# martinruenz/co-fusion

Measured on AMD Instinct MI355X. Metric: frames/sec at 640x480 (N active models) + ICP-reduce achieved HBM GB/s vs peak, higher is better.
Workload: dtype f32

## Files before the change

### co_fusion_amd/csrc/cf_device.h

```cpp
#pragma once

#include <hip/hip_runtime.h>
#include <stdint.h>

#include "cf_kernels.h"

namespace cf {

constexpr int kFixICP = 32;
constexpr int kFixRGB = 32;

__host__ __device__ inline int rgb_fix_bits(float sigma)
{
    if (sigma == -1.0f || !(sigma >= 2.0f)) return 8;
    union { float f; unsigned u; } v; v.f = sigma;
    const int F = 8 + 2 * ((int)((v.u >> 23) & 255u) - 127);
    return F > 32 ? 32 : F;
}
constexpr int kFixSO3 = 12;
constexpr int kSE3Words = 32;
constexpr int kSO3Words = 16;

struct f3 { float x, y, z; };
struct m33 { float m[9]; };
// ... 205 lines not shown

__device__ __forceinline__ void gram_wave_store(int* wl, const gram_v16i& acc, int lane)
{
#pragma unroll
    for (int g = 0; g < 4; g++)
#pragma unroll
        for (int a = 0; a < 3; a++) wl[(3 * g + a) * 64 + lane] = acc[4 * g + a];
}
__device__ __forceinline__ void gram_block_commit(const int* lds, bool has, int lane, int wave, int nwaves,
                                                  unsigned long long* __restrict__ dst )
{
    __shared__ int s_has[16];
    if (lane == 0) s_has[wave] = has ? 1 : 0;
    __syncthreads();
    if (wave != 0) return;
    gram_v16i c;
#pragma unroll
    for (int r = 0; r < 16; r++) c[r] = 0;
    bool any = false;
    for (int w = 0; w < nwaves; w++) {
        if (!s_has[w]) continue;
        any = true;
        const int* src = lds + w * kGramWaveDwords + lane;
#pragma unroll
        for (int g = 0; g < 4; g++)
#pragma unroll
            for (int a = 0; a < 3; a++) c[4 * g + a] += src[(3 * g + a) * 64];
    }
    if (!any) return;
    const unsigned long long v = gram_wave_finish(c, lane);
    const int word = gram_word_of_lane(lane);
    if (word >= 0 && v != 0) atomicAdd(&dst[word], v);
}

__device__ __forceinline__ void det_sincos(double x, double* s, double* c)
{
    const double two_over_pi = 0.63661977236758134308;
    const double pio2_1 = 1.57079632673412561417e+00;
    const double pio2_1t = 6.07710050650619224932e-11;
    double fn = rint(x * two_over_pi);
    double r = (x - fn * pio2_1) - fn * pio2_1t;
    long long n = (long long)fn;
    double r2 = r * r;
    double sp = -1.0 / 355687428096000.0;
    sp = sp * r2 + 1.0 / 1307674368000.0;
    sp = sp * r2 - 1.0 / 6227020800.0;
    sp = sp * r2 + 1.0 / 39916800.0;
    sp = sp * r2 - 1.0 / 362880.0;
    sp = sp * r2 + 1.0 / 5040.0;
    sp = sp * r2 - 1.0 / 120.0;
    sp = sp * r2 + 1.0 / 6.0;
    double sr = r - r * r2 * sp;
    double cp = 1.0 / 20922789888000.0;
    cp = cp * r2 - 1.0 / 87178291200.0;
    cp = cp * r2 + 1.0 / 479001600.0;
    cp = cp * r2 - 1.0 / 3628800.0;
    cp = cp * r2 + 1.0 / 40320.0;
    cp = cp * r2 - 1.0 / 720.0;
    cp = cp * r2 + 1.0 / 24.0;
    cp = cp * r2 - 1.0 / 2.0;
    double cr = 1.0 + r2 * cp;
    switch ((int)(n & 3)) {
        case 0: *s = sr; *c = cr; break;
        case 1: *s = cr; *c = -sr; break;
        case 2: *s = -sr; *c = -cr; break;
        default: *s = -cr; *c = sr; break;
    }
}

__device__ inline void rodrigues(const double w[3], double R[9])
{
    double rx = w[0], ry = w[1], rz = w[2];
    double theta = sqrt(rx * rx + ry * ry + rz * rz);
    R[0] = 1; R[1] = 0; R[2] = 0; R[3] = 0; R[4] = 1; R[5] = 0; R[6] = 0; R[7] = 0; R[8] = 1;
    if (theta >= 2.2204460492503131e-16) {
        double s, c;
        det_sincos(theta, &s, &c);
        double c1 = 1.0 - c;
        double itheta = 1.0 / theta;
        rx *= itheta; ry *= itheta; rz *= itheta;
        const double rrt[9] = {rx * rx, rx * ry, rx * rz, rx * ry, ry * ry, ry * rz, rx * rz, ry * rz, rz * rz};
        const double rx_[9] = {0, -rz, ry, rz, 0, -rx, -ry, rx, 0};
        const double I[9] = {1, 0, 0, 0, 1, 0, 0, 0, 1};
        for (int k = 0; k < 9; k++) R[k] = c * I[k] + c1 * rrt[k] + s * rx_[k];
    }
}

template <typename T>
__device__ inline void inv33(const T a[9], T o[9])
{
    T c00 = a[4] * a[8] - a[5] * a[7];
    T c01 = a[5] * a[6] - a[3] * a[8];
    T c02 = a[3] * a[7] - a[4] * a[6];
    T det = a[0] * c00 + a[1] * c01 + a[2] * c02;
    T id = (T)1 / det;
    o[0] = c00 * id;
    o[1] = (a[2] * a[7] - a[1] * a[8]) * id;
    o[2] = (a[1] * a[5] - a[2] * a[4]) * id;
    o[3] = c01 * id;
    o[4] = (a[0] * a[8] - a[2] * a[6]) * id;
    o[5] = (a[2] * a[3] - a[0] * a[5]) * id;
    o[6] = c02 * id;
    o[7] = (a[1] * a[6] - a[0] * a[7]) * id;
    o[8] = (a[0] * a[4] - a[1] * a[3]) * id;
}

template <typename T>
__device__ inline void mul33(const T a[9], const T b[9], T o[9])
{
    for (int i = 0; i < 3; i++)
        for (int j = 0; j < 3; j++)
            o[i * 3 + j] = a[i * 3 + 0] * b[0 * 3 + j] + a[i * 3 + 1] * b[1 * 3 + j] + a[i * 3 + 2] * b[2 * 3 + j];
}

__device__ inline void mul44(const double a[16], const double b[16], double o[16])
{
    for (int i = 0; i < 4; i++)
        for (int j = 0; j < 4; j++) {
            double s = a[i * 4 + 0] * b[0 * 4 + j];
            s = s + a[i * 4 + 1] * b[1 * 4 + j];
            s = s + a[i * 4 + 2] * b[2 * 4 + j];
            s = s + a[i * 4 + 3] * b[3 * 4 + j];
            o[i * 4 + j] = s;
        }
}

__device__ inline void inv44_affine(const double a[16], double o[16])
{
    double L[9] = {a[0], a[1], a[2], a[4], a[5], a[6], a[8], a[9], a[10]}, Li[9];
    inv33<double>(L, Li);
    for (int i = 0; i < 3; i++) {
        o[i * 4 + 0] = Li[i * 3 + 0]; o[i * 4 + 1] = Li[i * 3 + 1]; o[i * 4 + 2] = Li[i * 3 + 2];
        o[i * 4 + 3] = -(Li[i * 3 + 0] * a[3] + Li[i * 3 + 1] * a[7] + Li[i * 3 + 2] * a[11]);
    }
    o[12] = 0; o[13] = 0; o[14] = 0; o[15] = 1;
}

template <typename T, int N>
__device__ inline void ldlt_solve(const T* Ain, const T* b, T* x, T tiny, T* ws, int* iws)
{
    T* A = ws; T* y = ws + N * N; T* d = ws + N * N + N;
    int* perm = iws;
    for (int i = 0; i < N * N; i++) A[i] = Ain[i];
    for (int i = 0; i < N; i++) perm[i] = i;
    for (int k = 0; k < N; k++) {
        int p = k;
        T best = A[k * N + k] < 0 ? -A[k * N + k] : A[k * N + k];
        for (int i = k + 1; i < N; i++) {
            T v = A[i * N + i] < 0 ? -A[i * N + i] : A[i * N + i];
            if (v > best) { best = v; p = i; }
        }
        if (p != k) {
            for (int j = 0; j < N; j++) { T t = A[k * N + j]; A[k * N + j] = A[p * N + j]; A[p * N + j] = t; }
            for (int i = 0; i < N; i++) { T t = A[i * N + k]; A[i * N + k] = A[i * N + p]; A[i * N + p] = t; }
            int t = perm[k]; perm[k] = perm[p]; perm[p] = t;
        }
        T akk = A[k * N + k];
        d[k] = akk;
        T aabs = akk < 0 ? -akk : akk;
        if (aabs > tiny) {
            for (int i = k + 1; i < N; i++) A[i * N + k] = A[i * N + k] / akk;
            for (int i = k + 1; i < N; i++)
                for (int j = k + 1; j <= i; j++) {
                    A[i * N + j] = A[i * N + j] - A[i * N + k] * akk * A[j * N + k];
                    A[j * N + i] = A[i * N + j];
                }
        } else {
            for (int i = k + 1; i < N; i++) A[i * N + k] = 0;
        }
    }
    for (int i = 0; i < N; i++) {
        T s = b[perm[i]];
        for (int j = 0; j < i; j++) s = s - A[i * N + j] * y[j];
        y[i] = s;
    }
    for (int i = 0; i < N; i++) {
        T aabs = d[i] < 0 ? -d[i] : d[i];
        y[i] = (aabs > tiny) ? y[i] / d[i] : (T)0;
    }
    for (int i = N - 1; i >= 0; i--) {
        T s = y[i];
        for (int j = i + 1; j < N; j++) s = s - A[j * N + i] * y[j];
        y[i] = s;
    }
    for (int i = 0; i < N; i++) x[perm[i]] = y[i];
}

__device__ __forceinline__ double readlane_f64(double v, int lane)
{
    const int lo = __builtin_amdgcn_readlane(__double2loint(v), lane);
    const int hi = __builtin_amdgcn_readlane(__double2hiint(v), lane);
    return __hiloint2double(hi, lo);
}

__device__ __forceinline__ double bpermute_f64(double v, int byte_addr)
{
    const int lo = __builtin_amdgcn_ds_bpermute(byte_addr, __double2loint(v));
    const int hi = __builtin_amdgcn_ds_bpermute(byte_addr, __double2hiint(v));
    return __hiloint2double(hi, lo);
}
__device__ __forceinline__ void ldlt_solve6_wave(double a, double* x, double tiny, int lane)
{
    const bool isB = lane >= 36 && lane < 42;
    const int i = (lane < 36) ? lane / 6 : (isB ? lane - 36 : 0), j = (lane < 36) ? lane % 6 : (isB ? 6 : 0);
    int perm[6] = {0, 1, 2, 3, 4, 5};
    double d[6];
#pragma unroll
    for (int k = 0; k < 6; k++) {
        int p = 5;
        {
            double dq[6];
#pragma unroll
            for (int q = k; q < 6; q++) dq[q] = __builtin_fabs(readlane_f64(a, q * 7));
            double M = dq[k];
#pragma unroll
            for (int q = k + 1; q < 6; q++) M = __builtin_fmax(M, dq[q]);
#pragma unroll
            for (int q = 5; q >= k; q--) p = (dq[q] == M) ? q : p;
        }
        p = __builtin_amdgcn_readfirstlane(p);
        if (p != k) {
            const int si = (i == k) ? p : ((i == p) ? k : i), sj = (j == k) ? p : ((j == p) ? k : j);
            a = bpermute_f64(a, (isB ? 36 + si : (si > sj ? si : sj) * 6 + (si > sj ? sj : si)) * 4);
            const int pk = perm[k];
            int pp = pk;
#pragma unroll
            for (int q = k + 1; q < 6; q++)
                if (q == p) { pp = perm[q]; perm[q] = pk; }
            perm[k] = pp;
        }
        const double akk = readlane_f64(a, k * 7);
        d[k] = akk;
        const double aabs = akk < 0 ? -akk : akk;
        const bool pivot_ok = aabs > tiny;
        if (j == k && i > k) a = pivot_ok ? a / akk : 0.0;
        const double lik = bpermute_f64(a, (i * 6 + k) * 4);
        const double ljk = bpermute_f64(a, (j * 6 + k) * 4);
        const double yk = readlane_f64(a, 36 + k);
        if (isB) { if (i > k) a = a - lik * yk; }
        else if (pivot_ok && i > k && j > k && j <= i) a = a - lik * akk * ljk;
    }
    double y[6];
#pragma unroll
    for (int r = 0; r < 6; r++) y[r] = readlane_f64(a, 36 + r);
    {
        double yn = y[0], dn = d[0];
#pragma unroll
        for (int r = 1; r < 6; r++) if (lane == r) { yn = y[r]; dn = d[r]; }
        const double aabs = dn < 0 ? -dn : dn;
        const double q = (aabs > tiny) ? yn / dn : 0.0;
#pragma unroll
        for (int r = 0; r < 6; r++) y[r] = readlane_f64(q, r);
    }
#pragma unroll
    for (int r = 5; r >= 0; r--) {
        double s = y[r];
#pragma unroll
        for (int c = r + 1; c < 6; c++) s = s - readlane_f64(a, c * 6 + r) * y[c];
        y[r] = s;
    }
    if (lane == 0) {
#pragma unroll
        for (int r = 0; r < 6; r++) x[perm[r]] = y[r];
    }
}


__device__ __forceinline__ float fix_to_f32(long long q, int F) { return (float)ldexp((double)q, -F); }

}
// ... 1 lines not shown
```

### co_fusion_amd/csrc/track_reduce.hip

```cpp
#include "cf_device.h"
#include "cf_kernels.h"
#include "track_prep_dev.h"
#include "track_sums_dev.h"

namespace cf {

__device__ __forceinline__ int idiv(int n, IDiv d) { return (int)(__umulhi((unsigned)n, d.M) >> d.s); }

struct IcpProj { f3 vcurr_g; int g; int inb; int ux, uy; };

__device__ __forceinline__ IcpProj icp_project(const m33& Rcurr, const f3& tcurr, const m33& Rprev_inv, const f3& tprev, const cf_cam& intr,
                                               int cols, int rows, f3 vcurr)
{
    IcpProj o;
    o.vcurr_g = mul(Rcurr, vcurr) + tcurr;
    const f3 vcurr_cp = mul(Rprev_inv, o.vcurr_g - tprev);
    const int ux = f2i_rn(vcurr_cp.x * intr.fx / vcurr_cp.z + intr.cx);
    const int uy = f2i_rn(vcurr_cp.y * intr.fy / vcurr_cp.z + intr.cy);
    o.inb = !(ux < 0 || uy < 0 || ux >= cols || uy >= rows || vcurr_cp.z < 0);
    o.g = o.inb ? uy * cols + ux : 0;
    o.ux = o.inb ? ux : 0; o.uy = o.inb ? uy : 0;
    return o;
}

// ... 695 lines not shown
        gn.rgb_acc[m] = rgb_args[0].m[m].rgb_acc;
        gn.od_host[m] = h_states ? h_states[m] : nullptr;
    }
    const bool slots = mode != 0;
    bool any_culled = false;
    for (int m = 0; m < n; m++) any_culled = any_culled || (icp_args[0].m[m].cull && icp_args[0].m[m].err);
    const bool err_aside = icp && any_culled;
    bool hook_failed = false;
    for (int i = 2; i >= 0; i--) {
        const int N = (width >> i) * (height >> i);
        for (int j = 0; j < iterations[i]; j++) {
            const bool last_of_level = (j == iterations[i] - 1);
            int next_level = i;
            if (last_of_level) {
                next_level = i - 1;
                while (next_level >= 0 && iterations[next_level] == 0) next_level--;
            }
            RgbArgs ra = rgb_args[i];
            ra.compact = slots ? 1 : 0;
            ra.slot_px = cfg.threads * 4;
            {
                const bool timed = prof && prof->enabled && i == 0 && prof->used + 4 <= prof->capacity;
                IcpArgs a = icp_args[i];
                a.flags = (i == 0 && last_of_level) ? (err_aside ? 3 : 1) : 0;
                launch_icp_rgbres(s, cfg, a, ra, icp, rgb, n, i, timed ? prof->events[prof->used] : nullptr,
                                  timed ? prof->events[prof->used + 1] : nullptr);
                if (timed) {
                    prof->used += 2;
                    prof->bytes += (uint64_t)N * ((icp ? 24 + 24 * (uint64_t)n : 0) + (rgb ? (slots ? kRgbResidualBytesCompact : kRgbResidualBytes) * (uint64_t)n : 0));
                    prof->launches += 1;
                }
            }
            const bool err_here = err_aside && i == 0 && last_of_level;
            const bool err_with_step = err_here && rgb && slots && mode != 2;
            if (err_here && !err_with_step) {
                icp_error_surface_kernel<<<dim3((N + 255) / 256, n), 256, 0, s>>>(with_cdiv(icp_args[i]));
            }
            if (hook && hook->fn) {
                FoldArgs fa{}; int nf = 0;
                for (int m = 0; m < n; m++) if (hook->split[m]) fa.acc[nf++] = gn.icp_acc[m];
                if (nf) acc_fold_kernel<<<nf, 64, 0, s>>>(fa);
                for (int m = 0; m < n; m++)
                    if (hook->split[m] && hook->fn(hook->user, 0, gn.icp_acc[m], 32, (void*)s) != 0) hook_failed = true;
            }
            if (rgb && mode == 2) {
                const int n_slots = (N + ra.slot_px - 1) / ra.slot_px, n_quads = (n_slots + 1) / 2;
                rgb_step_solve_kernel<<<8 * n_quads * ((n + 7) / 8), 256, 0, s>>>(ra, so3_syncs, n_slots, n_quads, make_idiv(n_quads > 1 ? n_quads : 2), n,
                                                                                 cfg.gram ? -1 : kFixICP, next_level, last_of_level ? 1 : 0);
                continue;
            }
            if (rgb) {
                if (slots) {
                    const int n_slots = (N + ra.slot_px - 1) / ra.slot_px;
                    if (err_with_step) rgb_slot_step_err_kernel<<<dim3(n_slots + (N + 255) / 256, n), 256, 0, s>>>(ra, n_slots, with_cdiv(icp_args[i]));
                    else rgb_slot_step_kernel<<<dim3(n_slots, n), 256, 0, s>>>(ra, n_slots);
                }
                else rgb_step_kernel<<<dim3((N + 255) / 256, n), 256, 0, s>>>(ra);
            }
            gn_solve_kernel<<<n, 256, 0, s>>>(gn, next_level, last_of_level ? 1 : 0);
        }
    }
    return !hook_failed;
}

float replay_icp_level0(hipStream_t s, IcpLaunch cfg, const IcpArgs& a0, const RgbArgs& r0, int n, int slots, int ablate, int reps, hipEvent_t e0, hipEvent_t e1)
{
    IcpArgs a = a0; a.flags = ablate << 8;
    RgbArgs ra = r0; ra.compact = slots ? 1 : 0; ra.slot_px = cfg.threads * 4;
    for (int i = 0; i < 3; i++) launch_icp_rgbres(s, cfg, a, ra, true, true, n, 0, nullptr, nullptr);
    (void)hipEventRecord(e0, s);
    for (int i = 0; i < reps; i++) launch_icp_rgbres(s, cfg, a, ra, true, true, n, 0, nullptr, nullptr);
    (void)hipEventRecord(e1, s);
    (void)hipStreamSynchronize(s);
    float ms = 0; (void)hipEventElapsedTime(&ms, e0, e1);
    return ms * 1000.f / reps;
}

#ifdef CF_ABLATE
void trace_so3_dump(hipStream_t s)
{
    (void)hipStreamSynchronize(s);
    unsigned long long h[12][8];
    if (hipMemcpyFromSymbol(h, HIP_SYMBOL(g_so3_trace), sizeof(h)) != hipSuccess) return;
    fprintf(stderr, "[so3 trace] loop %lld ns\n", (long long)(h[11][1] - h[11][0]) * 10);
    for (int it = 0; it < 10; it++) {
        if (!h[it][0] || h[it][4] < h[it][0]) continue;
        fprintf(stderr, "[so3 trace] it %d: basis %5lld  pass %5lld  meeting %5lld  solve %5lld ns\n", it, (long long)(h[it][1] - h[it][0]) * 10,
                (long long)(h[it][2] - h[it][1]) * 10, (long long)(h[it][3] - h[it][2]) * 10, (long long)(h[it][4] - h[it][3]) * 10);
    }
    unsigned long long z[12][8] = {};
    (void)hipMemcpyToSymbol(HIP_SYMBOL(g_so3_trace), z, sizeof(z));
}
static unsigned long long* g_solve_trace_dev = nullptr;
void trace_solve_begin()
{
    if (!g_solve_trace_dev && hipMalloc(reinterpret_cast<void**>(&g_solve_trace_dev), 64 * 16 * 8) != hipSuccess) return;
    (void)hipMemset(g_solve_trace_dev, 0, 64 * 16 * 8);
    const unsigned zero = 0;
    (void)hipMemcpyToSymbol(HIP_SYMBOL(g_solve_iter), &zero, sizeof(zero));
    (void)hipMemcpyToSymbol(HIP_SYMBOL(g_solve_trace), &g_solve_trace_dev, sizeof(g_solve_trace_dev));
}
void trace_solve_end(hipStream_t s, const char* path)
{
    (void)hipStreamSynchronize(s);
    unsigned long long* none = nullptr;
    (void)hipMemcpyToSymbol(HIP_SYMBOL(g_solve_trace), &none, sizeof(none));
    if (!g_solve_trace_dev) return;
    std::vector<unsigned long long> h(64 * 16);
    (void)hipMemcpy(h.data(), g_solve_trace_dev, h.size() * 8, hipMemcpyDeviceToHost);
    FILE* f = fopen(path, "a");
    if (!f) return;
    fprintf(f, "# solve: ns from the kernel's first stamp -- loaded | totals | unpacked | LDLT | rodrigues | pose | next-iteration | write-back\n");
    for (int it = 0; it < 64; it++) {
        const unsigned long long* o = &h[(size_t)it * 16];
        if (!o[0]) continue;
        fprintf(f, "%2d", it);
        for (int k = 1; k <= 8; k++) fprintf(f, " %6lld", o[k] ? (long long)(o[k] - o[0]) * 10 : -1ll);
        fprintf(f, "\n");
    }
    fclose(f);
}
void trace_step_solve(hipStream_t s, IcpLaunch cfg, const IcpArgs& a0, const RgbArgs& r0, So3Sync* syncs, int n, const char* path)
{
    IcpArgs a = a0; a.flags = 0;
    RgbArgs ra = r0; ra.compact = 1; ra.slot_px = cfg.threads * 4;
    const int N = ra.cols * ra.rows, n_slots = (N + ra.slot_px - 1) / ra.slot_px, n_quads = (n_slots + 1) / 2, grid = 8 * n_quads * ((n + 7) / 8);
    unsigned long long* d = nullptr; unsigned long long* none = nullptr;
    if (hipMalloc(reinterpret_cast<void**>(&d), (size_t)grid * 64) != hipSuccess) return;
    FILE* f = fopen(path, "w");
    for (int rep = 0; rep < 3 && f; rep++) {
        (void)hipMemset(d, 0, (size_t)grid * 64);
        launch_icp_rgbres(s, cfg, a, ra, true, true, n, 0, nullptr, nullptr);
        (void)hipStreamSynchronize(s);
        (void)hipMemcpyToSymbol(HIP_SYMBOL(g_icp_trace), &d, sizeof(d));
        rgb_step_solve_kernel<<<grid, 256, 0, s>>>(ra, syncs, n_slots, n_quads, make_idiv(n_quads > 1 ? n_quads : 2), n, cfg.gram ? -1 : kFixICP, 0, 0);
        (void)hipStreamSynchronize(s);
        (void)hipMemcpyToSymbol(HIP_SYMBOL(g_icp_trace), &none, sizeof(none));
        std::vector<unsigned long long> h((size_t)grid * 8);
        (void)hipMemcpy(h.data(), d, h.size() * 8, hipMemcpyDeviceToHost);
        unsigned long long tmin = ~0ull;
        for (int b = 0; b < grid; b++) if (h[(size_t)b * 8] && h[(size_t)b * 8] < tmin) tmin = h[(size_t)b * 8];
        fprintf(f, "# rep %d grid %d trackers %d\n", rep, grid, n);
        for (int b = 0; b < grid; b++) {
            const unsigned long long* o = &h[(size_t)b * 8];
            if (!o[0] || o[5] == 0xffff) continue;
            auto rel = [&](unsigned long long t) { return t ? (long long)(t - tmin) * 10 : -1ll; };
            fprintf(f, "%d %d %lld %lld %lld %lld %lld\n", b, (int)o[5], rel(o[0]), rel(o[1]), rel(o[2]), rel(o[3]), rel(o[4]));
        }
    }
    if (f) fclose(f);
    (void)hipFree(d);
}
void trace_icp_level0(hipStream_t s, IcpLaunch cfg, const IcpArgs& a0, const RgbArgs& r0, int n, int slots, const char* path)
{
    IcpArgs a = a0; a.flags = 0;
    RgbArgs ra = r0; ra.compact = slots ? 1 : 0; ra.slot_px = cfg.threads * 4;
    unsigned long long* d = nullptr; unsigned long long* none = nullptr;
    const size_t cap = 1u << 16;
    if (hipMalloc(reinterpret_cast<void**>(&d), cap * 32) != hipSuccess) return;
    (void)hipMemset(d, 0, cap * 32);
    for (int i = 0; i < 2; i++) launch_icp_rgbres(s, cfg, a, ra, true, true, n, 0, nullptr, nullptr);
    (void)hipStreamSynchronize(s);
    (void)hipMemcpyToSymbol(HIP_SYMBOL(g_icp_trace), &d, sizeof(d));
    launch_icp_rgbres(s, cfg, a, ra, true, true, n, 0, nullptr, nullptr);
    (void)hipStreamSynchronize(s);
    (void)hipMemcpyToSymbol(HIP_SYMBOL(g_icp_trace), &none, sizeof(none));
    std::vector<unsigned long long> h((size_t)g_last_grid * 4);
    (void)hipMemcpy(h.data(), d, h.size() * 8, hipMemcpyDeviceToHost);
    (void)hipFree(d);
    FILE* f = fopen(path, "w");
    if (!f) return;
    unsigned long long tmin = ~0ull;
// ... 47 lines not shown
```

### co_fusion_amd/csrc/track_so3_dev.h

```cpp
#pragma once
#include "track_prep_dev.h"
#include "track_sums_dev.h"

namespace cf {

__device__ __forceinline__ void screen_box(const float* lo, const float* hi, const float* Rb, const float* tb, const float* Rcurr, const float* tcurr,
                                           cf_cam intr, float distThres, int W, int H, int lane, int (&out)[4], float (&zout)[2])
{
    const float finf = __int_as_float(0x7f800000);
    zout[0] = -finf; zout[1] = finf;
    if (!(lo[0] <= hi[0])) { out[0] = 1; out[1] = 1; out[2] = 0; out[3] = 0; return; }
    const float m = distThres * 1.01f + 1e-3f;
    const float px = (lane & 1) ? hi[0] + 3.f : lo[0] - 3.f, py = (lane & 2) ? hi[1] + 3.f : lo[1] - 3.f;
    const float znear = lo[2] - m, pz = (lane & 4) ? hi[2] + m : znear;
    const float cx_ = (px - intr.cx) / intr.fx * pz, cy_ = (py - intr.cy) / intr.fy * pz;
    const float dx = (Rb[0] * cx_ + Rb[1] * cy_ + Rb[2] * pz + tb[0]) - tcurr[0];
    const float dy = (Rb[3] * cx_ + Rb[4] * cy_ + Rb[5] * pz + tb[1]) - tcurr[1];
    const float dz = (Rb[6] * cx_ + Rb[7] * cy_ + Rb[8] * pz + tb[2]) - tcurr[2];
    const float xc = Rcurr[0] * dx + Rcurr[3] * dy + Rcurr[6] * dz;
    const float yc = Rcurr[1] * dx + Rcurr[4] * dy + Rcurr[7] * dz;
    const float zc = Rcurr[2] * dx + Rcurr[5] * dy + Rcurr[8] * dz;
    const float u = intr.fx * xc / zc + intr.cx, v = intr.fy * yc / zc + intr.cy;
    const bool bad = !(znear > 0.05f) || !(zc > 0.05f) || !is_finite(u) || !is_finite(v);
    float u0 = u, u1 = u, v0 = v, v1 = v, z0 = zc, z1 = zc;
#pragma unroll
    for (int o = 1; o < 8; o <<= 1) {
        u0 = fminf(u0, __shfl_xor(u0, o, 64)); u1 = fmaxf(u1, __shfl_xor(u1, o, 64));
        v0 = fminf(v0, __shfl_xor(v0, o, 64)); v1 = fmaxf(v1, __shfl_xor(v1, o, 64));
        z0 = fminf(z0, __shfl_xor(z0, o, 64)); z1 = fmaxf(z1, __shfl_xor(z1, o, 64));
    }
    if (__any(bad)) { out[0] = 0; out[1] = 0; out[2] = W - 1; out[3] = H - 1; return; }
    zout[0] = z0 - (1e-3f + 1e-3f * fabsf(z0)); zout[1] = z1 + (1e-3f + 1e-3f * fabsf(z1));
    const float fw = (float)(W + 16), fh = (float)(H + 16);
    out[0] = (int)floorf(fminf(fmaxf(u0, -16.f), fw)) - 3; out[1] = (int)floorf(fminf(fmaxf(v0, -16.f), fh)) - 3;
    out[2] = (int)ceilf(fminf(fmaxf(u1, -16.f), fw)) + 3; out[3] = (int)ceilf(fminf(fmaxf(v1, -16.f), fh)) + 3;
}

__device__ __forceinline__ void so3_gradient(const uint8_t* __restrict__ img, int cols, int x, int y, float& gx, float& gy)
{
    const float actu = (float)img[y * cols + x];
    float back = (float)img[y * cols + x - 1], fore = (float)img[y * cols + x + 1];
    gx = ((back + actu) / 2.0f) - ((fore + actu) / 2.0f);
    back = (float)img[(y - 1) * cols + x]; fore = (float)img[(y + 1) * cols + x];
    gy = ((back + actu) / 2.0f) - ((fore + actu) / 2.0f);
}

__device__ __forceinline__ void so3_pass(const uint8_t* __restrict__ lastImage, const uint8_t* __restrict__ nextImage,
                                         const m33& B, const m33& Ki, const float* __restrict__ krlr, int cols, int rows,
                                         unsigned long long (*lds)[16], unsigned long long* totals, int block, int blocks)
{
    constexpr float lim = (float)(1 << ((50 - kFixSO3) / 2));
    constexpr float scale = (float)(1 << kFixSO3);
    const int N = cols * rows, T = blockDim.x;
    unsigned long long acc[16];
#pragma unroll
    for (int k = 0; k < 16; k++) acc[k] = 0;
    const float a = krlr[0], b = krlr[1], c = krlr[2], d = krlr[3], e = krlr[4], f = krlr[5], g = krlr[6], h = krlr[7],
                ii = krlr[8];
    for (int k = block * T + threadIdx.x; k < N; k += blocks * T) {
        const int y = k / cols, x = k - y * cols;
        const f3 unwarped = {(float)x, (float)y, 1.0f};
        const f3 warped = mul(B, unwarped);
        const int wx = f2i_rn(warped.x / warped.z), wy = f2i_rn(warped.y / warped.z);
        if (!(wx >= 1 && wx < cols - 1 && wy >= 1 && wy < rows - 1 && x >= 1 && x < cols - 1 && y >= 1 && y < rows - 1))
            continue;
        float gnx, gny, glx, gly;
        so3_gradient(nextImage, cols, wx, wy, gnx, gny);
        so3_gradient(lastImage, cols, x, y, glx, gly);
        const float gx = (gnx + glx) / 2.0f, gy = (gny + gly) / 2.0f;
        const f3 point = mul(Ki, unwarped);
        const float z2 = point.z * point.z;
        const f3 left = {((point.z * (d * gy + a * gx)) - (gy * g * y) - (gx * g * x)) / z2,
                         ((point.z * (e * gy + b * gx)) - (gy * h * y) - (gx * h * x)) / z2,
                         ((point.z * (f * gy + c * gx)) - (gy * ii * y) - (gx * ii * x)) / z2};
        const f3 jac = cross(left, point);
        const float row[4] = {jac.x, jac.y, jac.z, -((float)nextImage[wy * cols + wx] - (float)lastImage[y * cols + x])};
        double r[4], rs[4];
#pragma unroll
        for (int q = 0; q < 4; q++) { r[q] = (double)clamp_row(row[q], lim); rs[q] = (double)(clamp_row(row[q], lim) * scale); }
#pragma unroll
        for (int p = 0; p < 3; p++)
#pragma unroll
            for (int q = 0; q < 4; q++)
                if (q >= p)
                    acc[4 * p - (p * (p - 1)) / 2 + (q - p)] += (unsigned long long)__double_as_longlong(fma(rs[p], r[q], kMagic)) - kMagicBits;
        acc[9] += (unsigned long long)__double_as_longlong(fma(rs[3], r[3], kMagic)) - kMagicBits;
        acc[10] += 1;
    }
    const int lane = threadIdx.x & 63, wave = threadIdx.x >> 6;
    const unsigned long long v = wave_reduce16_u64(acc, lane);
    if ((lane & 3) == 0) lds[wave][lane >> 2] = v;
    __syncthreads();
    if (threadIdx.x < 16) {
        unsigned long long t = 0;
        for (int w = 0; w < (T >> 6); w++) t += lds[w][threadIdx.x];
        totals[threadIdx.x] = t;
    }
    __syncthreads();
}

__device__ inline void so3_unpack(const unsigned long long* t, float A[9], float b[3], float residual[2])
{
    int shift = 0;
    for (int i = 0; i < 3; ++i)
        for (int j = i; j < 4; ++j) {
            const float value = fix_to_f32((long long)t[shift++], kFixSO3);
            if (j == 3) b[i] = value;
            else A[j * 3 + i] = A[i * 3 + j] = value;
        }
    residual[0] = fix_to_f32((long long)t[9], kFixSO3);
    residual[1] = (float)(long long)t[10];
}

__device__ inline void k_matrix(cf_cam c, double K[9])
{
    for (int i = 0; i < 9; i++) K[i] = 0;
    K[0] = c.fx; K[4] = c.fy; K[2] = c.cx; K[5] = c.cy; K[8] = 1;
}

__device__ inline void prepare_iteration(OdomDev* od, int level)
{
    double K[9], Kinv[9], Rt[16];
    k_matrix(cam_level(od->intr, level), K);
    inv33<double>(K, Kinv);
    inv44_affine(od->resultRt, Rt);
    const double R[9] = {Rt[0], Rt[1], Rt[2], Rt[4], Rt[5], Rt[6], Rt[8], Rt[9], Rt[10]};
    double tmp[9], KRK[9];
    mul33<double>(K, R, tmp);
    mul33<double>(tmp, Kinv, KRK);
    for (int k = 0; k < 9; k++) od->krkInv[k] = (float)KRK[k];
    const double tv[3] = {Rt[3], Rt[7], Rt[11]};
    for (int r = 0; r < 3; r++) od->kt[r] = (float)(K[r * 3 + 0] * tv[0] + K[r * 3 + 1] * tv[1] + K[r * 3 + 2] * tv[2]);
}

__global__ void __launch_bounds__(1024) so3_step_kernel(const uint8_t* __restrict__ lastImage,
                                                        const uint8_t* __restrict__ nextImage, m33 B, m33 Ki, m33 krlr,
                                                        int cols, int rows, unsigned long long* __restrict__ out16)
{
    __shared__ unsigned long long lds[16][16];
    __shared__ unsigned long long totals[16];
    so3_pass(lastImage, nextImage, B, Ki, krlr.m, cols, rows, lds, totals, blockIdx.x, gridDim.x);
    if (threadIdx.x < 16) out16[threadIdx.x] = totals[threadIdx.x];
}

#ifdef CF_ABLATE
__device__ unsigned long long g_so3_trace[12][8];
#define OSTAMP(it, k) do { if (lead && by == 0 && threadIdx.x == 0) g_so3_trace[it][k] = wall_clock64(); } while (0)
#else
#define OSTAMP(it, k) do {} while (0)
#endif
__global__ void __launch_bounds__(256) so3_prealign_kernel(const TrackerStates ts, So3Sync* __restrict__ syncs, int do_so3,
                                                           int first_level, int gx, int so3_blocks, const RgbPrepBatch prep, int prep_bx)
{
    if ((int)blockIdx.x >= so3_blocks) {
        const int r = (int)blockIdx.x - so3_blocks, m = r / prep_bx;
        rgb_prep_body(prep.m[m], r - m * prep_bx);
        return;
    }
    const int by = (int)blockIdx.x / gx, bxx = (int)blockIdx.x - by * gx;
    OdomDev* const god = ts.dev[by];
    So3Sync* sync = syncs + by;
    __shared__ OdomDev s_od;
    __shared__ unsigned long long lds[16][16];
    __shared__ unsigned long long totals[16];
    __shared__ float s_basis[9], s_kinv[9], s_krlr[9];
    __shared__ int s_done;
    __shared__ double s_resultR[9];
    __shared__ double s_K[9], s_Kinv[9];
    __shared__ float s_Rlr[9];
    __shared__ float s_lastError, s_lastCount;
    __shared__ double s_lastResultR[9];
    __shared__ float s_jtj[9], s_jtr[3], s_delta[3], s_fws[15];
    __shared__ int s_iws[3];
    const bool one_xcd = do_so3 && gx > 1;
    if (one_xcd && (bxx & 7) != (by & 7)) return;
    const int bx = one_xcd ? (bxx >> 3) : bxx;
    const bool lead = bx == 0;
    const unsigned G = one_xcd ? (unsigned)gx >> 3 : (unsigned)gx;
    {
        static_assert(sizeof(OdomDev) % 4 == 0, "OdomDev is staged as 32-bit words");
        constexpr int kWords = (int)(sizeof(OdomDev) / 4);
        const unsigned* __restrict__ src = reinterpret_cast<const unsigned*>(ts.host[by]);
        constexpr int kPer = (kWords + 255) / 256;
        unsigned w[kPer];
#pragma unroll
        for (int q = 0; q < kPer; q++) w[q] = ((int)threadIdx.x + 256 * q < kWords) ? src[threadIdx.x + 256 * q] : 0u;
#pragma unroll
        for (int q = 0; q < kPer; q++) if ((int)threadIdx.x + 256 * q < kWords) reinterpret_cast<unsigned*>(&s_od)[threadIdx.x + 256 * q] = w[q];
        __syncthreads();
        if (lead) for (int k = threadIdx.x; k < kWords; k += 256) reinterpret_cast<unsigned*>(god)[k] = reinterpret_cast<const unsigned*>(&s_od)[k];
        __syncthreads();
    }
    const OdomDev* const od = &s_od;
    const int L = 2, cols = od->width >> L, rows = od->height >> L;
    if (threadIdx.x == 0) {
        for (int k = 0; k < 9; k++) { s_resultR[k] = (k % 4 == 0) ? 1.0 : 0.0; s_lastResultR[k] = s_resultR[k]; s_Rlr[k] = (k % 4 == 0) ? 1.f : 0.f; }
        k_matrix(cam_level(od->intr, L), s_K);
        inv33<double>(s_K, s_Kinv);
        s_lastError = 3.402823466e+38F / 2; s_lastCount = 3.402823466e+38F / 2;
        s_done = 0;
        if (lead) { god->stats.so3_iterations = 0; god->stats.last_so3_error = 0; god->stats.last_so3_count = 0; }
    }
    __syncthreads();
    if (do_so3) {
        const uint8_t* __restrict__ lastNext = od->lastNextImage[L];
        const uint8_t* __restrict__ next = od->nextImage[L];
        OSTAMP(11, 0);
        for (int it = 0; it < 10; it++) {
            OSTAMP(it, 0);
            if (threadIdx.x == 0) {
                double tmp[9], H[9];
                mul33<double>(s_K, s_resultR, tmp);
                mul33<double>(tmp, s_Kinv, H);
                for (int k = 0; k < 9; k++) { s_basis[k] = (float)H[k]; s_kinv[k] = (float)s_Kinv[k]; s_krlr[k] = (float)tmp[k]; }
            }
            __syncthreads();
            m33 B, Ki;
            for (int k = 0; k < 9; k++) { B.m[k] = s_basis[k]; Ki.m[k] = s_kinv[k]; }
            OSTAMP(it, 1);
            so3_pass(lastNext, next, B, Ki, s_krlr, cols, rows, lds, totals, bx, (int)G);
            OSTAMP(it, 2);
            if (G > 1) {
                if (threadIdx.x < 64) {
                    unsigned long long* slot = sync->acc[it];
                    if (threadIdx.x < 11 && totals[threadIdx.x] != 0)
                        __hip_atomic_fetch_add(&slot[threadIdx.x], totals[threadIdx.x], __ATOMIC_RELAXED, __HIP_MEMORY_SCOPE_WORKGROUP);
                    asm volatile("s_waitcnt vmcnt(0)" ::: "memory");
                    if (threadIdx.x == 0) {
                        __hip_atomic_fetch_add(&sync->arrive, 1u, __ATOMIC_RELAXED, __HIP_MEMORY_SCOPE_WORKGROUP);
                        const unsigned target = (unsigned)(it + 1) * G;
                        unsigned spins = 0;
                        while (l2_read_u32(&sync->arrive) < target) {
                            if (++spins > (1u << 22)) { god->stats.fault = 1; break; }
                            __builtin_amdgcn_s_sleep(1);
                        }
                    }
                    __builtin_amdgcn_wave_barrier();
                    if (threadIdx.x < 16) totals[threadIdx.x] = l2_read_u64(&slot[threadIdx.x]);
                }
                __syncthreads();
            }
            OSTAMP(it, 3);
            if (threadIdx.x == 0) {
                float jtj[9], jtr[3], residual[2];
                so3_unpack(totals, jtj, jtr, residual);
                if (lead) god->stats.so3_iterations = it + 1;
                float err = sqrtf(residual[0]) / residual[1];
                float cnt = residual[1];
                if (err < s_lastError && (double)fabsf(s_lastError - cnt) < 0.001) {
                    s_done = 1;
                } else if ((double)err > (double)s_lastError + 0.001) {
                    err = s_lastError; cnt = s_lastCount;
                    for (int k = 0; k < 9; k++) s_resultR[k] = s_lastResultR[k];
                    s_done = 1;
                } else {
                    s_lastError = err; s_lastCount = cnt;
                    for (int k = 0; k < 9; k++) s_lastResultR[k] = s_resultR[k];
                    for (int k = 0; k < 9; k++) s_jtj[k] = jtj[k];
                    for (int k = 0; k < 3; k++) s_jtr[k] = jtr[k];
                    ldlt_solve<float, 3>(s_jtj, s_jtr, s_delta, 1.17549435e-38f, s_fws, s_iws);
                    const float delta[3] = {s_delta[0], s_delta[1], s_delta[2]};
                    const double dd[3] = {delta[0], delta[1], delta[2]};
                    double rotUpdate[9];
                    rodrigues(dd, rotUpdate);
                    float ru[9], nr[9];
                    for (int k = 0; k < 9; k++) ru[k] = (float)rotUpdate[k];
                    mul33<float>(ru, s_Rlr, nr);
                    for (int k = 0; k < 9; k++) { s_Rlr[k] = nr[k]; s_resultR[k] = nr[k]; }
                }
                if (lead) { god->stats.last_so3_error = err; god->stats.last_so3_count = cnt; }
            }
            __syncthreads();
            OSTAMP(it, 4);
            if (s_done) break;
        }
        OSTAMP(11, 1);
        if (G > 1 && threadIdx.x == 0) {
            if (__hip_atomic_fetch_add(&sync->depart, 1u, __ATOMIC_RELAXED, __HIP_MEMORY_SCOPE_WORKGROUP) == G - 1) {
                for (int it = 0; it < 10; it++)
                    for (int w = 0; w < 16; w++) sync->acc[it][w] = 0;
                sync->arrive = 0; sync->depart = 0;
            }
        }
    }
    if (lead && threadIdx.x < 64) {
        const int lane = threadIdx.x;
        unsigned key = 0;
        if (od->cull && lane < 6) { key = od->aabb_acc[lane]; od->aabb_acc[lane] = 0; }
        const float val = lane < 3 ? fkey_inv(~key) : fkey_inv(key);
        float lo[3], hi[3];
#pragma unroll
        for (int k = 0; k < 3; k++) { lo[k] = __shfl(val, k, 64); hi[k] = __shfl(val, 3 + k, 64); }
        if (__shfl((int)key, 3, 64) == 0) { lo[0] = 1.f; hi[0] = 0.f; }
        int ib[4] = {0, 0, od->width - 1, od->height - 1};
        float zb[2] = {-__int_as_float(0x7f800000), __int_as_float(0x7f800000)};
        if (od->cull) screen_box(lo, hi, od->box_R, od->box_t, od->Rcurr, od->tcurr, od->intr, od->distThres, od->width, od->height, lane, ib, zb);
        if (lane == 0) {
            for (int k = 0; k < 3; k++) { god->box_lo[k] = lo[k]; god->box_hi[k] = hi[k]; }
            for (int k = 0; k < 4; k++) god->stats.cull_box[k] = ib[k];
            god->cull_z[0] = zb[0]; god->cull_z[1] = zb[1];
        }
    }
    if (lead && threadIdx.x == 0) {
        for (int k = 0; k < 16; k++) god->resultRt[k] = (k % 5 == 0) ? 1.0 : 0.0;
        if (do_so3)
            for (int x = 0; x < 3; x++)
                for (int y = 0; y < 3; y++) god->resultRt[x * 4 + y] = s_resultR[x * 3 + y];
        god->lastRGBError = 3.402823466e+38F;
        god->level_done = 0;
        god->residual[0] = 0; god->residual[1] = 0;
        prepare_iteration(god, first_level);
        refresh_hot(god);
    }
}

}
```

Before: 916.3.

## Keep SO3 prealign state in registers and drop per-iteration serial basis step

The SO3 prealignment loop now keeps the rotation, last error and K matrices in per-thread registers of the first wave instead of shared memory. The basis update is folded into the solve step, which removes one __syncthreads and a serial thread-0 phase per iteration. A branch-free 3x3 LDLT replaces the generic shared-memory solver. The epilogue builds the hot state directly instead of re-reading global memory. It also adds trace instrumentation for prologue/epilogue timing and per-tracker iteration counts under CF_ABLATE. The risk is subtle numerical or ordering differences, for example with the sync reset that moved to the end of the kernel.

New measurement: 898.9. -1.9%, worse.

```diff
diff --git a/co_fusion_amd/csrc/cf_device.h b/co_fusion_amd/csrc/cf_device.h
--- a/co_fusion_amd/csrc/cf_device.h
+++ b/co_fusion_amd/csrc/cf_device.h
@@ -311,6 +311,7 @@
         const double rrt[9] = {rx * rx, rx * ry, rx * rz, rx * ry, ry * ry, ry * rz, rx * rz, ry * rz, rz * rz};
         const double rx_[9] = {0, -rz, ry, rz, 0, -rx, -ry, rx, 0};
         const double I[9] = {1, 0, 0, 0, 1, 0, 0, 0, 1};
+#pragma unroll
         for (int k = 0; k < 9; k++) R[k] = c * I[k] + c1 * rrt[k] + s * rx_[k];
     }
 }
@@ -337,7 +338,9 @@
 template <typename T>
 __device__ inline void mul33(const T a[9], const T b[9], T o[9])
 {
+#pragma unroll
     for (int i = 0; i < 3; i++)
+#pragma unroll
         for (int j = 0; j < 3; j++)
             o[i * 3 + j] = a[i * 3 + 0] * b[0 * 3 + j] + a[i * 3 + 1] * b[1 * 3 + j] + a[i * 3 + 2] * b[2 * 3 + j];
 }
@@ -358,6 +361,7 @@
 {
     double L[9] = {a[0], a[1], a[2], a[4], a[5], a[6], a[8], a[9], a[10]}, Li[9];
     inv33<double>(L, Li);
+#pragma unroll
     for (int i = 0; i < 3; i++) {
         o[i * 4 + 0] = Li[i * 3 + 0]; o[i * 4 + 1] = Li[i * 3 + 1]; o[i * 4 + 2] = Li[i * 3 + 2];
         o[i * 4 + 3] = -(Li[i * 3 + 0] * a[3] + Li[i * 3 + 1] * a[7] + Li[i * 3 + 2] * a[11]);
@@ -415,6 +419,62 @@
     for (int i = 0; i < N; i++) x[perm[i]] = y[i];
 }
 
+__device__ __forceinline__ void ldlt_solve3(const float (&A)[9], const float (&b)[3], float (&x)[3], float tiny)
+{
+    auto mag = [](float v) { return v < 0 ? -v : v; };
+    const float a00 = A[0], a01 = A[1], a02 = A[2], a10 = A[3], a11 = A[4], a12 = A[5], a20 = A[6], a21 = A[7], a22 = A[8];
+    const float b0 = b[0], b1 = b[1], b2 = b[2];
+    int p = 0;
+    float best = mag(a00);
+    if (mag(a11) > best) { best = mag(a11); p = 1; }
+    if (mag(a22) > best) p = 2;
+    float d0 = p == 0 ? a00 : (p == 1 ? a11 : a22);
+    float d1 = p == 1 ? a00 : a11;
+    float d2 = p == 2 ? a00 : a22;
+    float l10 = p == 0 ? a10 : (p == 1 ? a01 : a12);
+    float l20 = p == 0 ? a20 : (p == 1 ? a21 : a02);
+    float l21 = p == 0 ? a21 : (p == 1 ? a20 : a01);
+    int perm0 = p, perm1 = p == 1 ? 0 : 1, perm2 = p == 2 ? 0 : 2;
+    const float D0 = d0;
+    const bool ok0 = mag(D0) > tiny;
+    {
+        const float q10 = l10 / D0, q20 = l20 / D0;
+        const float n11 = d1 - q10 * D0 * q10, n21 = l21 - q20 * D0 * q10, n22 = d2 - q20 * D0 * q20;
+        l10 = ok0 ? q10 : 0.f; l20 = ok0 ? q20 : 0.f;
+        d1 = ok0 ? n11 : d1; l21 = ok0 ? n21 : l21; d2 = ok0 ? n22 : d2;
+    }
+    if (mag(d2) > mag(d1)) {
+        float t = d1; d1 = d2; d2 = t;
+        t = l10; l10 = l20; l20 = t;
+        const int ti = perm1; perm1 = perm2; perm2 = ti;
+    }
+    const float D1 = d1;
+    const bool ok1 = mag(D1) > tiny;
+    {
+        const float q21 = l21 / D1;
+        const float n22 = d2 - q21 * D1 * q21;
+        l21 = ok1 ? q21 : 0.f;
+        d2 = ok1 ? n22 : d2;
+    }
+    const float D2 = d2;
+    const bool ok2 = mag(D2) > tiny;
+    float y0 = perm0 == 0 ? b0 : (perm0 == 1 ? b1 : b2);
+    float y1 = perm1 == 0 ? b0 : (perm1 == 1 ? b1 : b2);
+    float y2 = perm2 == 0 ? b0 : (perm2 == 1 ? b1 : b2);
+    y1 = y1 - l10 * y0;
+    y2 = y2 - l20 * y0;
+    y2 = y2 - l21 * y1;
+    y0 = ok0 ? y0 / D0 : 0.f;
+    y1 = ok1 ? y1 / D1 : 0.f;
+    y2 = ok2 ? y2 / D2 : 0.f;
+    y1 = y1 - l21 * y2;
+    y0 = y0 - l10 * y1;
+    y0 = y0 - l20 * y2;
+    x[0] = perm0 == 0 ? y0 : (perm1 == 0 ? y1 : y2);
+    x[1] = perm0 == 1 ? y0 : (perm1 == 1 ? y1 : y2);
+    x[2] = perm0 == 2 ? y0 : (perm1 == 2 ? y1 : y2);
+}
+
 __device__ __forceinline__ double readlane_f64(double v, int lane)
 {
     const int lo = __builtin_amdgcn_readlane(__double2loint(v), lane);
diff --git a/co_fusion_amd/csrc/track_reduce.hip b/co_fusion_amd/csrc/track_reduce.hip
--- a/co_fusion_amd/csrc/track_reduce.hip
+++ b/co_fusion_amd/csrc/track_reduce.hip
@@ -801,12 +801,21 @@
     (void)hipStreamSynchronize(s);
     unsigned long long h[12][8];
     if (hipMemcpyFromSymbol(h, HIP_SYMBOL(g_so3_trace), sizeof(h)) != hipSuccess) return;
-    fprintf(stderr, "[so3 trace] loop %lld ns\n", (long long)(h[11][1] - h[11][0]) * 10);
+    fprintf(stderr, "[so3 trace] prologue %lld  loop %lld  epilogue %lld ns\n", (long long)(h[11][0] - h[11][2]) * 10, (long long)(h[11][1] - h[11][0]) * 10,
+            (long long)(h[11][3] - h[11][1]) * 10);
     for (int it = 0; it < 10; it++) {
         if (!h[it][0] || h[it][4] < h[it][0]) continue;
         fprintf(stderr, "[so3 trace] it %d: basis %5lld  pass %5lld  meeting %5lld  solve %5lld ns\n", it, (long long)(h[it][1] - h[it][0]) * 10,
                 (long long)(h[it][2] - h[it][1]) * 10, (long long)(h[it][3] - h[it][2]) * 10, (long long)(h[it][4] - h[it][3]) * 10);
     }
+    int iters[kMaxBatch];
+    if (hipMemcpyFromSymbol(iters, HIP_SYMBOL(g_so3_iters), sizeof(iters)) == hipSuccess) {
+        fprintf(stderr, "[so3 trace] iterations per tracker:");
+        for (int m = 0; m < kMaxBatch; m++) fprintf(stderr, " %d", iters[m]);
+        fprintf(stderr, "\n");
+    }
+    int zi[kMaxBatch] = {};
+    (void)hipMemcpyToSymbol(HIP_SYMBOL(g_so3_iters), zi, sizeof(zi));
     unsigned long long z[12][8] = {};
     (void)hipMemcpyToSymbol(HIP_SYMBOL(g_so3_trace), z, sizeof(z));
 }
diff --git a/co_fusion_amd/csrc/track_so3_dev.h b/co_fusion_amd/csrc/track_so3_dev.h
--- a/co_fusion_amd/csrc/track_so3_dev.h
+++ b/co_fusion_amd/csrc/track_so3_dev.h
@@ -99,10 +99,12 @@
     __syncthreads();
 }
 
-__device__ inline void so3_unpack(const unsigned long long* t, float A[9], float b[3], float residual[2])
+__device__ __forceinline__ void so3_unpack(const unsigned long long* t, float A[9], float b[3], float residual[2])
 {
     int shift = 0;
+#pragma unroll
     for (int i = 0; i < 3; ++i)
+#pragma unroll
         for (int j = i; j < 4; ++j) {
             const float value = fix_to_f32((long long)t[shift++], kFixSO3);
             if (j == 3) b[i] = value;
@@ -114,23 +116,9 @@
 
 __device__ inline void k_matrix(cf_cam c, double K[9])
 {
+#pragma unroll
     for (int i = 0; i < 9; i++) K[i] = 0;
     K[0] = c.fx; K[4] = c.fy; K[2] = c.cx; K[5] = c.cy; K[8] = 1;
-}
-
-__device__ inline void prepare_iteration(OdomDev* od, int level)
-{
-    double K[9], Kinv[9], Rt[16];
-    k_matrix(cam_level(od->intr, level), K);
-    inv33<double>(K, Kinv);
-    inv44_affine(od->resultRt, Rt);
-    const double R[9] = {Rt[0], Rt[1], Rt[2], Rt[4], Rt[5], Rt[6], Rt[8], Rt[9], Rt[10]};
-    double tmp[9], KRK[9];
-    mul33<double>(K, R, tmp);
-    mul33<double>(tmp, Kinv, KRK);
-    for (int k = 0; k < 9; k++) od->krkInv[k] = (float)KRK[k];
-    const double tv[3] = {Rt[3], Rt[7], Rt[11]};
-    for (int r = 0; r < 3; r++) od->kt[r] = (float)(K[r * 3 + 0] * tv[0] + K[r * 3 + 1] * tv[1] + K[r * 3 + 2] * tv[2]);
 }
 
 __global__ void __launch_bounds__(1024) so3_step_kernel(const uint8_t* __restrict__ lastImage,
@@ -145,9 +133,12 @@
 
 #ifdef CF_ABLATE
 __device__ unsigned long long g_so3_trace[12][8];
+__device__ int g_so3_iters[kMaxBatch];
+#define OITERS(n) do { g_so3_iters[by] = (n); } while (0)
 #define OSTAMP(it, k) do { if (lead && by == 0 && threadIdx.x == 0) g_so3_trace[it][k] = wall_clock64(); } while (0)
 #else
 #define OSTAMP(it, k) do {} while (0)
+#define OITERS(n) do {} while (0)
 #endif
 __global__ void __launch_bounds__(256) so3_prealign_kernel(const TrackerStates ts, So3Sync* __restrict__ syncs, int do_so3,
                                                            int first_level, int gx, int so3_blocks, const RgbPrepBatch prep, int prep_bx)
@@ -165,18 +156,28 @@
     __shared__ unsigned long long totals[16];
     __shared__ float s_basis[9], s_kinv[9], s_krlr[9];
     __shared__ int s_done;
-    __shared__ double s_resultR[9];
-    __shared__ double s_K[9], s_Kinv[9];
-    __shared__ float s_Rlr[9];
-    __shared__ float s_lastError, s_lastCount;
-    __shared__ double s_lastResultR[9];
-    __shared__ float s_jtj[9], s_jtr[3], s_delta[3], s_fws[15];
-    __shared__ int s_iws[3];
     const bool one_xcd = do_so3 && gx > 1;
     if (one_xcd && (bxx & 7) != (by & 7)) return;
     const int bx = one_xcd ? (bxx >> 3) : bxx;
     const bool lead = bx == 0;
     const unsigned G = one_xcd ? (unsigned)gx >> 3 : (unsigned)gx;
+    OSTAMP(11, 2);
+    float R[9] = {1.f, 0.f, 0.f, 0.f, 1.f, 0.f, 0.f, 0.f, 1.f}, lastR[9] = {1.f, 0.f, 0.f, 0.f, 1.f, 0.f, 0.f, 0.f, 1.f};
+    float lastError = 3.402823466e+38F / 2, lastCount = 3.402823466e+38F / 2;
+    double K[9], Kinv[9];
+    int so3_iterations = 0;
+    float so3_error = 0, so3_count = 0;
+    auto publish = [&](const float (&Rf)[9]) {
+        double Rd[9], tmp[9], H[9];
+#pragma unroll
+        for (int k = 0; k < 9; k++) Rd[k] = (double)Rf[k];
+        mul33<double>(K, Rd, tmp);
+        mul33<double>(tmp, Kinv, H);
+        if (threadIdx.x == 0) {
+#pragma unroll
+            for (int k = 0; k < 9; k++) { s_basis[k] = (float)H[k]; s_krlr[k] = (float)tmp[k]; }
+        }
+    };
     {
         static_assert(sizeof(OdomDev) % 4 == 0, "OdomDev is staged as 32-bit words");
         constexpr int kWords = (int)(sizeof(OdomDev) / 4);
@@ -189,18 +190,21 @@
         for (int q = 0; q < kPer; q++) if ((int)threadIdx.x + 256 * q < kWords) reinterpret_cast<unsigned*>(&s_od)[threadIdx.x + 256 * q] = w[q];
         __syncthreads();
         if (lead) for (int k = threadIdx.x; k < kWords; k += 256) reinterpret_cast<unsigned*>(god)[k] = reinterpret_cast<const unsigned*>(&s_od)[k];
-        __syncthreads();
     }
     const OdomDev* const od = &s_od;
     const int L = 2, cols = od->width >> L, rows = od->height >> L;
-    if (threadIdx.x == 0) {
-        for (int k = 0; k < 9; k++) { s_resultR[k] = (k % 4 == 0) ? 1.0 : 0.0; s_lastResultR[k] = s_resultR[k]; s_Rlr[k] = (k % 4 == 0) ? 1.f : 0.f; }
-        k_matrix(cam_level(od->intr, L), s_K);
-        inv33<double>(s_K, s_Kinv);
-        s_lastError = 3.402823466e+38F / 2; s_lastCount = 3.402823466e+38F / 2;
-        s_done = 0;
-        if (lead) { god->stats.so3_iterations = 0; god->stats.last_so3_error = 0; god->stats.last_so3_count = 0; }
-    }
+    if (do_so3 && threadIdx.x < 64) {
+        k_matrix(cam_level(od->intr, L), K);
+        inv33<double>(K, Kinv);
+        publish(R);
+        if (threadIdx.x == 0) {
+#pragma unroll
+            for (int k = 0; k < 9; k++) s_kinv[k] = (float)Kinv[k];
+            s_done = 0;
+        }
+    }
+    unsigned key = 0;
+    if (lead && od->cull && threadIdx.x < 6) key = od->aabb_acc[threadIdx.x];
     __syncthreads();
     if (do_so3) {
         const uint8_t* __restrict__ lastNext = od->lastNextImage[L];
@@ -208,13 +212,6 @@
         OSTAMP(11, 0);
         for (int it = 0; it < 10; it++) {
             OSTAMP(it, 0);
-            if (threadIdx.x == 0) {
-                double tmp[9], H[9];
-                mul33<double>(s_K, s_resultR, tmp);
-                mul33<double>(tmp, s_Kinv, H);
-                for (int k = 0; k < 9; k++) { s_basis[k] = (float)H[k]; s_kinv[k] = (float)s_Kinv[k]; s_krlr[k] = (float)tmp[k]; }
-            }
-            __syncthreads();
             m33 B, Ki;
             for (int k = 0; k < 9; k++) { B.m[k] = s_basis[k]; Ki.m[k] = s_kinv[k]; }
             OSTAMP(it, 1);
@@ -241,52 +238,49 @@
                 __syncthreads();
             }
             OSTAMP(it, 3);
-            if (threadIdx.x == 0) {
+            if (threadIdx.x < 64) {
                 float jtj[9], jtr[3], residual[2];
                 so3_unpack(totals, jtj, jtr, residual);
-                if (lead) god->stats.so3_iterations = it + 1;
+                so3_iterations = it + 1;
                 float err = sqrtf(residual[0]) / residual[1];
                 float cnt = residual[1];
-                if (err < s_lastError && (double)fabsf(s_lastError - cnt) < 0.001) {
-                    s_done = 1;
-                } else if ((double)err > (double)s_lastError + 0.001) {
-                    err = s_lastError; cnt = s_lastCount;
-                    for (int k = 0; k < 9; k++) s_resultR[k] = s_lastResultR[k];
-                    s_done = 1;
+                int done = 0;
+                if (err < lastError && (double)fabsf(lastError - cnt) < 0.001) {
+                    done = 1;
+                } else if ((double)err > (double)lastError + 0.001) {
+                    err = lastError; cnt = lastCount;
+#pragma unroll
+                    for (int k = 0; k < 9; k++) R[k] = lastR[k];
+                    done = 1;
                 } else {
-                    s_lastError = err; s_lastCount = cnt;
-                    for (int k = 0; k < 9; k++) s_lastResultR[k] = s_resultR[k];
-                    for (int k = 0; k < 9; k++) s_jtj[k] = jtj[k];
-                    for (int k = 0; k < 3; k++) s_jtr[k] = jtr[k];
-                    ldlt_solve<float, 3>(s_jtj, s_jtr, s_delta, 1.17549435e-38f, s_fws, s_iws);
-                    const float delta[3] = {s_delta[0], s_delta[1], s_delta[2]};
+                    lastError = err; lastCount = cnt;
+#pragma unroll
+                    for (int k = 0; k < 9; k++) lastR[k] = R[k];
+                    float delta[3];
+                    ldlt_solve3(jtj, jtr, delta, 1.17549435e-38f);
                     const double dd[3] = {delta[0], delta[1], delta[2]};
                     double rotUpdate[9];
                     rodrigues(dd, rotUpdate);
                     float ru[9], nr[9];
+#pragma unroll
                     for (int k = 0; k < 9; k++) ru[k] = (float)rotUpdate[k];
-                    mul33<float>(ru, s_Rlr, nr);
-                    for (int k = 0; k < 9; k++) { s_Rlr[k] = nr[k]; s_resultR[k] = nr[k]; }
+                    mul33<float>(ru, R, nr);
+#pragma unroll
+                    for (int k = 0; k < 9; k++) R[k] = nr[k];
+                    if (it < 9) publish(R);
                 }
-                if (lead) { god->stats.last_so3_error = err; god->stats.last_so3_count = cnt; }
+                so3_error = err; so3_count = cnt;
+                if (threadIdx.x == 0) s_done = done;
             }
             __syncthreads();
             OSTAMP(it, 4);
             if (s_done) break;
         }
         OSTAMP(11, 1);
-        if (G > 1 && threadIdx.x == 0) {
-            if (__hip_atomic_fetch_add(&sync->depart, 1u, __ATOMIC_RELAXED, __HIP_MEMORY_SCOPE_WORKGROUP) == G - 1) {
-                for (int it = 0; it < 10; it++)
-                    for (int w = 0; w < 16; w++) sync->acc[it][w] = 0;
-                sync->arrive = 0; sync->depart = 0;
-            }
-        }
     }
     if (lead && threadIdx.x < 64) {
         const int lane = threadIdx.x;
-        unsigned key = 0;
-        if (od->cull && lane < 6) { key = od->aabb_acc[lane]; od->aabb_acc[lane] = 0; }
+        if (od->cull && lane < 6) od->aabb_acc[lane] = 0;
         const float val = lane < 3 ? fkey_inv(~key) : fkey_inv(key);
         float lo[3], hi[3];
 #pragma unroll
@@ -299,19 +293,58 @@
             for (int k = 0; k < 3; k++) { god->box_lo[k] = lo[k]; god->box_hi[k] = hi[k]; }
             for (int k = 0; k < 4; k++) god->stats.cull_box[k] = ib[k];
             god->cull_z[0] = zb[0]; god->cull_z[1] = zb[1];
-        }
-    }
-    if (lead && threadIdx.x == 0) {
-        for (int k = 0; k < 16; k++) god->resultRt[k] = (k % 5 == 0) ? 1.0 : 0.0;
-        if (do_so3)
-            for (int x = 0; x < 3; x++)
-                for (int y = 0; y < 3; y++) god->resultRt[x * 4 + y] = s_resultR[x * 3 + y];
-        god->lastRGBError = 3.402823466e+38F;
-        god->level_done = 0;
-        god->residual[0] = 0; god->residual[1] = 0;
-        prepare_iteration(god, first_level);
-        refresh_hot(god);
-    }
-}
-
-}
+            god->stats.so3_iterations = so3_iterations; god->stats.last_so3_error = so3_error; god->stats.last_so3_count = so3_count;
+            OITERS(so3_iterations);
+            double Rt0[16];
+#pragma unroll
+            for (int k = 0; k < 16; k++) Rt0[k] = (k % 5 == 0) ? 1.0 : 0.0;
+            if (do_so3) {
+#pragma unroll
+                for (int x = 0; x < 3; x++)
+#pragma unroll
+                    for (int y = 0; y < 3; y++) Rt0[x * 4 + y] = (double)R[x * 3 + y];
+            }
+#pragma unroll
+            for (int k = 0; k < 16; k++) god->resultRt[k] = Rt0[k];
+            god->lastRGBError = 3.402823466e+38F;
+            god->level_done = 0;
+            god->residual[0] = 0; god->residual[1] = 0;
+            double K1[9], K1inv[9], Rt[16];
+            k_matrix(cam_level(od->intr, first_level), K1);
+            inv33<double>(K1, K1inv);
+            inv44_affine(Rt0, Rt);
+            const double Rn[9] = {Rt[0], Rt[1], Rt[2], Rt[4], Rt[5], Rt[6], Rt[8], Rt[9], Rt[10]};
+            double tmp[9], KRK[9];
+            mul33<double>(K1, Rn, tmp);
+            mul33<double>(tmp, K1inv, KRK);
+            const double tv[3] = {Rt[3], Rt[7], Rt[11]};
+            GnHot h;
+            h.icp = od->icp; h.level_done = 0; h.cull_z[0] = zb[0]; h.cull_z[1] = zb[1];
+#pragma unroll
+            for (int k = 0; k < 9; k++) { h.Rcurr[k] = od->Rcurr[k]; h.Rprev_inv[k] = od->Rprev_inv[k]; h.krkInv[k] = (float)KRK[k]; }
+#pragma unroll
+            for (int r = 0; r < 3; r++) {
+                h.tcurr[r] = od->tcurr[r]; h.tprev[r] = od->tprev[r];
+                h.kt[r] = (float)(K1[r * 3 + 0] * tv[0] + K1[r * 3 + 1] * tv[1] + K1[r * 3 + 2] * tv[2]);
+            }
+#pragma unroll
+            for (int k = 0; k < 4; k++) h.cull_box[k] = ib[k];
+            h.rgb = od->rgb; h.rgbOnly = od->rgbOnly; h.level_done2 = 0; h.pad = 0;
+#pragma unroll
+            for (int k = 0; k < 9; k++) god->krkInv[k] = h.krkInv[k];
+#pragma unroll
+            for (int r = 0; r < 3; r++) god->kt[r] = h.kt[r];
+            god->hot = h;
+        }
+    }
+    if (do_so3 && G > 1 && threadIdx.x == 0) {
+        if (__hip_atomic_fetch_add(&sync->depart, 1u, __ATOMIC_RELAXED, __HIP_MEMORY_SCOPE_WORKGROUP) == G - 1) {
+            for (int it = 0; it < 10; it++)
+                for (int w = 0; w < 16; w++) sync->acc[it][w] = 0;
+            sync->arrive = 0; sync->depart = 0;
+        }
+    }
+    OSTAMP(11, 3);
+}
+
+}
```
